# moss-lab/ScanFold

Hardware: AMD Instinct MI355X
Metric: windows/sec (W=120, step=1, 100 shuffles) (higher is better)
Workload: dtype int32 (int16 LDS storage) energies; f64 partition function

## Files before the change

### scanfold_amd/csrc/scanfold_hip.hip

```cpp
#include <math.h>
#include <stddef.h>
#include <stdio.h>
#include <stdlib.h>
#include <string.h>

#include <algorithm>
#include <map>
#include <string>
#include <vector>

#include "../../include/scanfold_hip_long.h"
#include "sf_launch.h"
#include "sf_energy.h"
#include "sf_mfe_full.hip.h"
#include "sf_mfe_fast.hip.h"
#include "sf_mfe_long.hip.h"
#include "sf_pf.hip.h"
#include "sf_pf_long.hip.h"
#include "sf_pf_fast.hip.h"
#include "sf_pf_lds.hip.h"
#include "sf_shuffle.hip.h"
#include "sf_tabulate.hip.h"
#include "sf_duplex.hip.h"

// ... 918 lines not shown
  return SF_OK;
}

int sf_last_status(void) {
  SF_ENTER();
  return read_status(nullptr, true);
}

int sf_set_max_bp_span(int span) {
  SF_ENTER();
  g.max_bp_span = span > 0 ? span : 0;
  if (g.have_params) {
    const int32_t md = g.max_bp_span > 0 ? g.max_bp_span - 1 : 0x7fffffff;
    HIPCHK(hipStreamSynchronize(g.stream));
    HIPCHK(hipMemcpy((char *)g.dP + offsetof(SfDevParams, max_pair_dist), &md, sizeof md, hipMemcpyHostToDevice));
    g.slot[g.cur].span = g.max_bp_span;
  }
  return SF_OK;
}

int sf_set_kernel_mode(int mode) {
  SF_ENTER();
  if (mode < 0 || mode > 1) return SF_ERR_BAD_ARG;
  g.force_full = (mode == 1);
  return SF_OK;
}


int sf_prof_reset(void) {
  SF_ENTER();
  HIPCHK(hipDeviceSynchronize());
  for (auto &e : g.ev) { hipEventDestroy(e.first); hipEventDestroy(e.second); }
  g.ev.clear();
  g.prof_ms = 0.0;
  g.prof_launches = 0;
  g.prof_folds = 0;
  g.prof_on = true;
  return SF_OK;
}

int sf_prof_get(double *ms, int64_t *launches, int64_t *folds) {
  SF_ENTER();
  HIPCHK(hipDeviceSynchronize());
  ProfPair::prof_drain();
  if (ms) *ms = g.prof_ms;
  if (launches) *launches = g.prof_launches;
  if (folds) *folds = g.prof_folds;
  return SF_OK;
}

int sf_prof_stop(void) {
  SF_ENTER();
  g.prof_on = false;
  return SF_OK;
}

}

namespace {
double g_long_ms[3] = {0, 0, 0};

struct LongBufs {
  std::vector<void *> ptrs;
  hipEvent_t ev[4] = {nullptr, nullptr, nullptr, nullptr};
  const char *who = "sf_fold_long";
  ~LongBufs() {
    hipStreamSynchronize(g.stream);
    for (void *p : ptrs) hipFree(p);
    for (hipEvent_t e : ev)
      if (e) hipEventDestroy(e);
  }
  int alloc(void **p, size_t bytes, const char *what) {
    *p = nullptr;
    const hipError_t e = hipMalloc(p, bytes ? bytes : 1);
    if (e != hipSuccess) {
      hipGetLastError();
      char b[512];
      snprintf(b, sizeof b, "%s: hipMalloc of %zu bytes (%s) failed: %s", who, bytes, what, hipGetErrorString(e));
      g.last_hip_error = b;
      *p = nullptr;
      return SF_ERR_HIP;
    }
    ptrs.push_back(*p);
    return SF_OK;
  }
};

int long_group(int d) {
  int G = 1;
  while (G < 64 && G * 64 < d) G *= 2;
  return G;
}
}

extern "C" {

int sf_fold_long(const uint8_t *seq, int L, const char *cons, int32_t *mfe_out, char *db_out) {
  int rc = check_ready();
  if (rc) return rc;
  if (!seq || L < 1 || L > SF_MAX_LONG) return SF_ERR_BAD_ARG;
  bool noncanonical = false;
  if (cons && (rc = scan_constraints(seq, cons, 1, L, &noncanonical))) return rc;
  const sf_params_blob *P = (const sf_params_blob *)g.slot[g.cur].src.data();
  std::vector<uint8_t> hS((size_t)L + 2, 0);
  for (int x = 0; x < L; x++) hS[x + 1] = sf_encode_nt(seq[x]);
  std::vector<int32_t> hhp((size_t)L + 1);
// ... 543 lines not shown
```

### scanfold_amd/csrc/sf_mfe_fast.hip.h

```cpp
#pragma once
#include <type_traits>
#include "sf_energy.h"
#include "sf_pk16.h"

#define SF_FAST_NR 34
#ifndef SF_FAST_TINY_D0
#define SF_FAST_TINY_D0 10
#endif
#define SF_FAST_CHUNK_D0 36
#ifndef SF_FAST_UNPACK
#define SF_FAST_UNPACK 1
#endif
#ifndef SF_UNP_PB
#define SF_UNP_PB 4
#endif
#define SF_HELP_MERGE_MAXW 118
#define SF_DML_HELPER_BIAS_256 26
#define SF_DML_HELPER_BIAS_W200 50
#define SF_DML_HELPER_BIAS(ng, wt) ((ng) == 256 ? ((wt) == 200 ? SF_DML_HELPER_BIAS_W200 : SF_DML_HELPER_BIAS_256) : 100000)
#define SF_HELP_NB_128 4
#define SF_HELP_NB_128G 8
#define SF_HELP_NB_256 6
#define SF_INF16 30000
#define SF_FAST_THRESH 10000
// ... 689 lines not shown
    if (!FOLD && slotd == 0) X.CI[SF_FAST_NR * RW + i0] = X.CI[rbd];
    const uint32_t bn = sf_pk(c + tau_in, c + X.t1n[SF_TIDX(tr, sq1, sp1)]);
    sf_fast_publish_bn(X.BN + 2 * rbd, i0, bn);
    if (X.bn_dup && slotd == 0) sf_fast_publish_bn(X.BN + 2 * (SF_FAST_NR * RW + i0), i0, bn);
    int stem, ext;
    if (i > 1 && j < W) { stem = X.tM[SF_TIDX(type, sp1, sq1)]; ext = X.tE[SF_TIDX(type, sp1, sq1)]; }
    else if (i > 1) stem = ext = X.tD5[type * 5 + sp1];
    else if (j < W) stem = ext = X.tD3[type * 5 + sq1];
    else stem = ext = 0;
    f = c + stem + tau_in + X.MLintern;
    cx = sfd_min(c + ext + tau_in, SF_INF16);
  } else {
    X.CI[rbd] = SF_INF16; sf_fast_publish_bn(X.BN + 2 * rbd, i0, sf_pk(SF_INF16, SF_INF16));
    if (!FOLD && slotd == 0) X.CI[SF_FAST_NR * RW + i0] = SF_INF16;
    if (X.bn_dup && slotd == 0) sf_fast_publish_bn(X.BN + 2 * (SF_FAST_NR * RW + i0), i0, sf_pk(SF_INF16, SF_INF16));
  }
  X.cg[SF_CGIDX(i, j)] = (int16_t)cx;
  if (final_fml && d > SFD_TURN + 1) f = sfd_min(f, fnb);
  if ((SEC & SF_SEC_DML) && (SEC & SF_SEC_FIN)) multiloop_split();
  f = sfd_min(f, dec);
  dprev = dec > SF_FAST_THRESH ? SF_INF16 : dec;
  fpart = f;
  if (final_fml && f < SF_FAST_OVF) ovf = 1;
  X.fML[FBASE(d) + i0] = (int16_t)(f > SF_FAST_THRESH ? SF_INF16 : f);
#undef ROW
#undef ROWB_CI
#undef ROWB_BN
#undef CIROW
#undef BNROWB
}

__device__ __forceinline__ int sf_wave_min(int v) {
#ifdef SF_EMUL
  return sfemul_wave_min(v);
#else
  v = sfd_min(v, __builtin_amdgcn_update_dpp(v, v, 0xB1, 0xF, 0xF, false));
  v = sfd_min(v, __builtin_amdgcn_update_dpp(v, v, 0x4E, 0xF, 0xF, false));
  v = sfd_min(v, __builtin_amdgcn_update_dpp(v, v, 0x141, 0xF, 0xF, false));
  v = sfd_min(v, __builtin_amdgcn_update_dpp(v, v, 0x140, 0xF, 0xF, false));
  v = sfd_min(v, __builtin_amdgcn_update_dpp(v, v, 0x142, 0xA, 0xF, false));
  v = sfd_min(v, __builtin_amdgcn_update_dpp(v, v, 0x143, 0xC, 0xF, false));
  return __builtin_amdgcn_readlane(v, 63);
#endif
}

__device__ __forceinline__ uint32_t sf_wave_next(uint32_t v) {
#ifdef SF_EMUL
  return __shfl_down(v, 1);
#else
  return (uint32_t)__builtin_amdgcn_update_dpp(0, (int)v, 0x130, 0xF, 0xF, true);
#endif
}

template <int WT, int LGC = 0>
__device__ __forceinline__ int sf_fast_dml2(const SfFastCtx &X, const int d, const int lane, const int i_own, const bool valid) {
  constexpr bool FOLD = false;
  const int W = WT ? WT : X.W;
  const int n = W - d, npairs = (n + 1) >> 1;
  const int lg = LGC ? LGC : (npairs <= 7 ? 3 : (npairs <= 15 ? 4 : 5));
  const int NC = 64 >> lg;
  const int q = lane & ((1 << lg) - 1), c = lane >> lg;
  const int elast = (d & 1) ? d - 6 : d - 5;
  const int N = elast - 3;
  const int S = (((N + NC - 1) >> (6 - lg)) + 1) & ~1;
  const int T8 = (S + 7) & ~7;
  const int ms = sfd_min(4 + c * S, elast - T8 + 1);
  const int ys = d - 1 - ms;
  const int par_a = W & 1, M0 = W - ys, par_b = (W - d + 1) & 1;
  const char *pa = (const char *)(X.fML + FBASE(ms) + 2 * q) - 36;
  const char *pb = (const char *)(X.fML + FBASE(ys) + 2 * q + ms + 1) - 64;
  int sa0 = 2 * (W - ms + par_a), sa1 = sa0 - 4 * par_a;
  int sb0 = 2 * (M0 - 1 - par_b), sb1 = 2 * (M0 - 1 + par_b);
  uint32_t acc0 = sf_pk(32767, 32767), acc1 = acc0;
  for (int t = 0; t < T8; t += 8) {
    uint32_t wa[8], wb[8];
#pragma unroll
    for (int k = 0; k < 8; k++) {
      constexpr int E[8] = {0, 0, 0, 2, 4, 8, 12, 18}, G2[8] = {0, 2, 4, 8, 12, 18, 24, 32};
      wa[k] = sf_ldw((const int16_t *)(pa + (36 - 2 * E[k])));
      wb[k] = sf_ldw((const int16_t *)(pb + (64 - 2 * G2[k] - ((k & 1) ? 0 : 2))));
      pa += (k & 1) ? (k < 7 ? sa1 : sa1 - 48) : sa0;
      pb -= (k & 1) ? (k < 7 ? sb1 : sb1 + 80) : sb0;
    }
    sa0 -= 16; sa1 -= 16; sb0 += 16; sb1 += 16;
#pragma unroll
    for (int k = 0; k < 8; k++) {
      uint32_t b = wb[k];
      if (!(k & 1)) b = (sf_wave_next(b) << 16) | (b >> 16);
      if (k & 1) acc1 = sf_pkmin(acc1, sf_pkadd(wa[k], b)); else acc0 = sf_pkmin(acc0, sf_pkadd(wa[k], b));
    }
  }
  if (d & 1) {
    const uint32_t a = sf_ldw(X.fML + FBASE(d - 5) + 2 * q);
    const uint32_t w = sf_ldw(X.fML + 2 * q + d - 5);
    acc0 = sf_pkmin(acc0, sf_pkadd(a, (sf_wave_next(w) << 16) | (w >> 16)));
  }
  uint32_t acc = sf_pkmin(acc0, acc1);
  acc = sf_pkmin_xor32(acc);
  if (lg <= 4) acc = sf_pkmin_xor16(acc);
  if (lg <= 3) acc = sf_pkmin_xor8(acc);
  const int i0 = valid ? i_own - 1 : 0;
  const uint32_t r = __shfl(acc, i0 >> 1);
  return (i0 & 1) ? sf_hi(r) : sf_lo(r);
}

__device__ __forceinline__ int sf_fast_c(const SfFastCtx &X, const int16_t *tExt, const int i, const int j) {
  const int W = X.W;
  const int v = X.cg[SF_CGIDX(i, j)];
  if (!X.cg_ext || v >= SF_INF16) return v;
  const uint8_t *S = X.S;
  const int type = X.tPair[S[i] * 8 + S[j]];
  int ext;
  if (i > 1 && j < W) ext = tExt[SF_TIDX(type, S[i - 1], S[j + 1])];
  else if (i > 1) ext = X.tD5[type * 5 + S[i - 1]];
  else if (j < W) ext = X.tD3[type * 5 + S[j + 1]];
  else ext = 0;
  return v - ext - (type > 2 ? X.TAU : 0);
}

__device__ inline int sf_fast_traceback(const SfFastCtx &X, const int32_t *f5s, const int16_t *tExt, const int lane,
                                        int16_t *stI, int16_t *stJ, int16_t *stM, char *dbL) {
  const int W = X.W;
  const bool FOLD = X.fold != 0;
  const uint8_t *S = X.S;
  const SfDevParams *D = X.D;
#define TC(i, j) sf_fast_c(X, tExt, (i), (j))
#define TF(i, j) (((j) - (i) < SFD_TURN + 1) ? SF_INF16 : (int)X.fML[FBASE((j) - (i)) + (i)-1])
#define TPAIR(i, j) (((j) - (i)) <= X.maxd ? (int)X.tPair[S[i] * 8 + S[j]] : 0)
  for (int x = lane; x < W; x += 64) dbL[x] = '.';
  int sp = 0, bad = 0;
  stI[0] = 1; stJ[0] = (int16_t)W; stM[0] = 0; sp = 1;
  while (sp > 0 && !bad) {
    --sp;
    int i = stI[sp], j = stJ[sp];
    const int ml = stM[sp];
    bool have_pair = false;
    if (ml == 0) {
      while (j > 0 && f5s[j] == f5s[j - 1]) j--;
      if (j < SFD_TURN + 2) continue;
      const int fij = f5s[j];
      int found = -1;
      for (int base = j - SFD_TURN - 1; base >= 1 && found < 0; base -= 64) {
        const int k = base - lane;
        bool ok = false;
        if (k >= 1) {
          const int type = TPAIR(k, j);
          if (type) {
            int ext;
            if (k > 1 && j < W) ext = tExt[SF_TIDX(type, S[k - 1], S[j + 1])];
            else if (k > 1) ext = X.tD5[type * 5 + S[k - 1]];
            else if (j < W) ext = X.tD3[type * 5 + S[j + 1]];
            else ext = 0;
            ok = (fij == f5s[k - 1] + TC(k, j) + ext + (type > 2 ? X.TAU : 0));
          }
        }
// ... 194 lines not shown
    if (bad && lane == 0) atomicOr(status, 1);
  }
}

#define SF_DEFER_ROWS_256 3
template <int NQ>
struct SfTrail {
  int F[NQ];
  int f3n;
  int row;
};
template <int NQ>
__device__ __forceinline__ void sf_trail_load(const int16_t *cgp, const int W, const int lane, const int i, int (&c)[NQ]) {
#pragma unroll
  for (int q = 0; q < NQ; q++) {
    const int j = lane + 1 + 64 * q;
    c[q] = (i >= 1 && j <= W && i + SFD_TURN + 1 <= j) ? (int)cgp[SF_CGIDX(i, j)] : SF_INF16;
  }
}
template <int NQ>
__device__ __forceinline__ void sf_trail_row(SfTrail<NQ> &T, const int lane, const int i, const int (&c)[NQ]) {
  if (i < 1) return;
  int m = c[0] + T.F[0];
#pragma unroll
  for (int q = 1; q < NQ; q++) m = sfd_min(m, c[q] + T.F[q]);
  T.f3n = sfd_min(T.f3n, sf_wave_min(m));
  if (i >= 2) {
    const int l = (i - 2) & 63, h = (i - 2) >> 6;
#pragma unroll
    for (int q = 0; q < NQ; q++) T.F[q] = (lane == l && h == q) ? T.f3n : T.F[q];
  }
}
template <int NQ, int NR>
__device__ __forceinline__ void sf_trail_rows(SfTrail<NQ> &T, const int lane, const int nrows, const int (&c)[NR][NQ]) {
#pragma unroll
  for (int k = 0; k < NR; k++)
    if (k < nrows) sf_trail_row<NQ>(T, lane, T.row - k, c[k]);
  T.row -= nrows;
}
template <int NQ>
__device__ __forceinline__ void sf_trail_result(const SfTrail<NQ> &T, const int lane, const int seq, const int over,
                                                int32_t *__restrict__ out, int *__restrict__ ovf_cnt,
                                                int *__restrict__ ovf_list) {
  if (lane == 0) {
    out[seq] = T.f3n;
    if (over || T.f3n < SF_FAST_OVF) {
      const int k = atomicAdd(ovf_cnt, 1);
      ovf_list[k] = seq;
    }
  }
}


enum SfStep {
  SF_STEP_SIZED,
  SF_STEP_GUARDED,
  SF_STEP_UNSPLIT,
  SF_STEP_SPLIT,
  SF_STEP_SPLIT16,
  SF_STEP_SPLIT8,
  SF_STEP_NARROW,
};
template <SfStep K>
using SfStepTag = std::integral_constant<SfStep, K>;

__device__ __forceinline__ int16_t sf_poison16(const int poison, const int x) {
  const int k = poison == 5 ? 1 + (int)(((uint32_t)x * 2654435761u) >> 30) : poison;
  return (int16_t)(k == 1 ? -32768 : (k == 2 ? -28000 : (k == 3 ? 0 : 32767)));
}

template <int NG, int WT, bool MG = false, bool HC = false, bool PZ = false>
__global__ __launch_bounds__(2 * NG, SF_FAST_WAVES_PER_SIMD) void sf_mfe_fast_kernel(const uint8_t *__restrict__ seqs, int n, int Wrt,
                                                             const SfDevParams *__restrict__ D,
                                                             const SfFastParams *__restrict__ F,
                                                             const SfFastRows *__restrict__ Rows,
                                                             int16_t *__restrict__ cg_all, int32_t *__restrict__ out,
                                                             int *__restrict__ ovf_cnt, int *__restrict__ ovf_list,
                                                             int trace_stride, char *__restrict__ db_out,
                                                             int *__restrict__ status, int *__restrict__ work_ctr,
                                                             const char *__restrict__ cons_rows,
                                                             const int32_t *__restrict__ sc_rows, int poison) {
  constexpr int NT = 2 * NG;
  constexpr bool FOLD = (NG == 256);
  const int W = WT ? WT : Wrt;
  SF_DYN_SMEM(smem);
  const SfFastLayout Lo = sf_fast_layout(W, HC);
  SfFastCtx X;
  char *const hcC = (char *)(smem + Lo.off_hc);
  uint8_t *const hcP = (uint8_t *)hcC + (W + 2), *const hcE = hcP + (W + 2);
  int16_t *const scS = (int16_t *)(smem + Lo.off_hc + (((3 * (W + 2)) + 1) & ~1));
  X.hc.c = (HC && cons_rows) ? hcC : nullptr; X.hc.partner = hcP; X.hc.encl = hcE;
  X.sc = (HC && sc_rows) ? scS : nullptr;
  X.fML = (int16_t *)smem;
  X.CI = (int16_t *)(smem + Lo.off_ci);
  X.C1N = nullptr; X.CB = nullptr;
  X.BN = (int16_t *)(smem + Lo.off_c1n);
#ifdef SF_EMUL
  sf_emul_bn_base = (const char *)X.BN; sf_emul_ci_base = (const char *)X.CI;
#endif
  X.DMLr = nullptr;
  int16_t *tab = (int16_t *)(smem + Lo.off_tab);
  X.t23 = tab; X.tI = tab + 175 - 25; X.t1n = tab + 325 - 25; X.tM = tab + 475 - 25; X.tH = tab + 625 - 25;
  X.tE = tab + 775 - 25; X.cg_ext = 1;
  X.tStack = tab + 925; X.tD5 = tab + 989; X.tD3 = tab + 1029;
  uint8_t *tPair = (uint8_t *)(tab + 1069);
  X.tPair = tPair;
  uint8_t *tRPair = (uint8_t *)(tab + SF_FAST_TAB_OLD);
  int16_t *t23in = tab + SF_FAST_TAB_OLD + 32;
  X.tRPair = tRPair; X.t23in = t23in;
  int32_t *flag = (int32_t *)(smem + Lo.off_flag);
  uint8_t *S = (uint8_t *)(smem + Lo.off_S);
  X.S = S;
  X.D = D; X.F = F; X.R = Rows; X.W = W; X.fold = FOLD; X.maxd = D->max_pair_dist;
  constexpr bool MERGE = MG && (NG == 128);
  constexpr bool UNPK = SF_FAST_UNPACK && (NG == 128);
  constexpr bool LGLOOPS = MG && (NG == 128);
  constexpr int TBLK = WT > 0 ? 1 : (NG == 128 ? (MG ? 2 : 1) : 0);
  X.bn_dup = (NG == 128);
  uint8_t *const cell_list = (MG && W >= SF_HELP_MERGE_MAXW) ? (uint8_t *)((int16_t *)(smem + Lo.off_tab) + 1069 + 32 + 1)
                                                            : (uint8_t *)(smem + Lo.off_list);
  X.TAU = D->P.TerminalAU; X.MLbase = D->P.MLbase; X.MLclosing = D->P.MLclosing; X.MLintern = D->P.MLintern[1];
  int32_t *f5s = (int32_t *)(smem + Lo.off_ci);
  int16_t *tExt = (int16_t *)(smem + Lo.off_ci + (((W + 1) * 4 + 3) & ~3));

  const int tid = threadIdx.x;
  X.cg = cg_all + (size_t)sf_fast_scratch_slot(blockIdx.x, gridDim.x) * SF_CG_ENTRIES(W);
  for (int x = tid; x < 175; x += NT) {
    tab[x] = F->mm23[x];
    if (x < 150) {
      tab[175 + x] = F->mmI[25 + x]; tab[325 + x] = F->mm1n[25 + x]; tab[475 + x] = F->mmM[25 + x];
      tab[625 + x] = F->mmH[25 + x]; tab[775 + x] = F->mmExt[25 + x];
    }
  }
  for (int x = tid; x < 175; x += NT) t23in[x] = F->mm23in[x];
  for (int x = tid; x < 64; x += NT) { tab[925 + x] = F->stackT[x]; tPair[x] = F->pair[x]; tRPair[x] = F->rpair[x]; }
  for (int x = tid; x < 40; x += NT) { tab[989 + x] = F->d5[x]; tab[1029 + x] = F->d3[x]; }

  {
    int16_t *uni = tab + 1069 + 32 + 1;
    X.uNIN = uni;
    for (int x = tid; x < 128; x += NT) uni[x] = F->uni[x];
  }
  const int grp = SF_WAVE_UNIFORM(tid / NG);
  const int tg = tid - grp * NG;
  constexpr int CENTRE = (NG == 256) ? 128 : 32;
  constexpr bool SHARE = SF_DML_HELPER_BIAS(NG, WT) < 10000;
  constexpr bool DML2 = (NG == 128);
  const int OFFs = ((W + 1) >> 1) - CENTRE;
  const int OFF = (NG > 64) ? (OFFs + NG) & (NG - 1) : 0;
  const int v = (tg + OFF) & (NG - 1);
  constexpr int MAIN_LO = (NG == 256) ? 64 : 0, MAIN_HI = (NG == 256) ? 191 : 63;
  const bool can_split = (NG == 128 && W >= 64) || NG == 256;
  const int split_d0 = can_split ? ((sfd_max(sfd_max(SFD_MAXLOOP + 6, 2 * (MAIN_LO - 1 + OFFs)), 2 * (W - OFFs - MAIN_HI)) + 1) & ~1) : 1 << 30;
  constexpr bool NARROW = (NG == 256);
  const int narrow_d0 = (NARROW && can_split && W >= 168)
                            ? sfd_max(split_d0, (sfd_max(2 * (96 - 1 + OFFs), 2 * (W - OFFs - 159)) + 1) & ~1) : 1 << 30;

  constexpr int NQ = NG / 64;
  const bool sweeper = SF_WAVE_UNIFORM(tid >> 6) == (NG == 128 ? 3 : 7);
  const int n_split_steps = split_d0 < W ? (W - split_d0 + 1) / 2 : 0;
  constexpr int DROWS = (NG == 128 || WT != 200) ? 4 : SF_DEFER_ROWS_256;
  const int defer_need = n_split_steps > 0 ? (W - SFD_TURN - 1 + n_split_steps - 1) / n_split_steps : 0;
  const int defer_rows = sfd_min(defer_need, DROWS);
  const bool defer_on = n_split_steps >= 8 && defer_need <= 4;
  SfTrail<NQ> T;
#pragma unroll
  for (int q = 0; q < NQ; q++) T.F[q] = 0;
  T.f3n = 0; T.row = 0;

  int *const next_slot = (int *)(smem + Lo.off_next);
  int seq = blockIdx.x;
  while (seq < n) {
    const uint8_t *src = seqs + (size_t)seq * W;
    constexpr bool PINF = true;
    int tidf = tid;
    if (PINF) SF_PIN(tidf);
    __syncthreads();
    if (PZ) {
      for (int x = tid; x < Lo.off_tab / 2; x += NT) ((int16_t *)smem)[x] = sf_poison16(poison, x);
      if (HC) for (int x = tid; x < (Lo.total - Lo.off_hc) / 2; x += NT) ((int16_t *)(smem + Lo.off_hc))[x] = sf_poison16(poison, x);
      __syncthreads();
    }
    for (int x = tidf; x < W; x += NT) S[x + 1] = sf_encode_nt(src[x]);
    if (MG && W >= SF_HELP_MERGE_MAXW) for (int x = tidf; x < 128; x += NT) ((int16_t *)(smem + Lo.off_tab) + 1069 + 32 + 1)[x] = F->uni[x];
    for (int x = tidf; x < (Lo.off_tab - Lo.off_ci) / 4; x += NT) ((uint32_t *)X.CI)[x] = sf_pk(SF_INF16, SF_INF16);
    int fetched = 0;
    if (tid == 0) {
      S[0] = 0; S[W + 1] = 0; flag[0] = 0;
      fetched = (int)gridDim.x + atomicAdd(work_ctr, 1);
    }
    __syncthreads();
    if (HC) {
      if (cons_rows)
        for (int x = tid; x < W; x += NT) hcC[x + 1] = cons_rows[(size_t)seq * W + x];
      if (sc_rows)
        for (int x = tid; x < W; x += NT) scS[x + 1] = (int16_t)sfd_max(sfd_min(sc_rows[(size_t)seq * W + x], 30000), -30000);
      __syncthreads();
      if (cons_rows && tid == 0) flag[0] = sf_hc_parse8(W, hcC, hcP, hcE) ? 2 : 0;
      __syncthreads();
      if (cons_rows && flag[0] == 2) {
        if (tid == 0) { atomicOr(status, 2); out[seq] = 0; *next_slot = fetched; }
        __syncthreads();
        seq = *next_slot;
        continue;
      }
    }
    int next_seq = n;
    const bool trail_this = defer_on && !(db_out && (seq % trace_stride) == 0);
    if (sweeper) {
#pragma unroll
      for (int q = 0; q < NQ; q++) T.F[q] = 0;
      T.f3n = 0; T.row = trail_this ? W - SFD_TURN - 1 : 0;
    }
    int ovf = 0;
    uint32_t H[14];
    int dprev = SF_INF16;
    int fnb = SF_FAST_BIG;
#pragma unroll
    for (int k = 0; k < 14; k++) H[k] = (uint32_t)SF_INF16 | ((uint32_t)SF_INF16 << 16);

    int slot2 = (SFD_TURN + 1 + grp - 2) % SF_FAST_NR, slotd = (SFD_TURN + 1 + grp) % SF_FAST_NR;
    auto build_list = [&](const int dd0) {
      const int lane = tid & 63;
      const int d1 = dd0 + 1;
      const int iH = ((v - 64) & (NG - 1)) - (dd0 >> 1);
      const bool vA = (dd0 < W) && (iH >= 1) && (iH + dd0 <= W), vB = (d1 < W) && (iH >= 1) && (iH + d1 <= W);
      const int tA = (vA && dd0 <= X.maxd) ? X.tPair[S[iH] * 8 + S[iH + dd0]] : 0;
      const int tB = (vB && d1 <= X.maxd) ? X.tPair[S[iH] * 8 + S[iH + d1]] : 0;
      const unsigned long long mA = __ballot(tA != 0), mB = __ballot(tB != 0);
      const int cA = __popcll(mA);
      uint8_t *list = cell_list + (((dd0 >> 1) & 1) << 7);
      const unsigned long long below = (1ull << lane) - 1ull;
      if (tA) list[__popcll(mA & below)] = (uint8_t)iH;
      if (tB) list[cA + __popcll(mB & below)] = (uint8_t)(iH | 128);
      if (lane == 0) list[127] = (uint8_t)(cA + __popcll(mB));
    };
    SfHU HU;
    auto step = [&](const int d0, auto kind_tag) {
      constexpr SfStep KIND = decltype(kind_tag)::value;
      constexpr int LGC = KIND == SF_STEP_SPLIT16 ? 4 : (KIND == SF_STEP_SPLIT8 ? 3 : (KIND == SF_STEP_SPLIT && LGLOOPS ? 5 : 0));
      constexpr bool DO_G = KIND == SF_STEP_SIZED, DO_CH = KIND == SF_STEP_GUARDED;
      const int d = d0 + grp;
      if (d0 == SFD_TURN + 1 + 2 && tid == 0) *next_slot = fetched;
      if (d0 == SFD_TURN + 1 + 4) next_seq = SF_WAVE_UNIFORM(*next_slot);
      constexpr bool split = KIND >= SF_STEP_SPLIT;
      constexpr bool narrow = KIND == SF_STEP_NARROW;
      if (NARROW && d0 == narrow_d0) {
        uint32_t *const xa = (uint32_t *)X.BN;
        const int RWc = W - 4;
        if (tg >= 96 && tg < 160) {
#pragma unroll
          for (int k = 0; k < 14; k++) xa[(grp * 16 + k) * RWc + 100 + (tg - 96)] = H[k];
          xa[(grp * 16 + 14) * RWc + 100 + (tg - 96)] = (uint32_t)dprev;
          xa[(grp * 16 + 15) * RWc + 100 + (tg - 96)] = (uint32_t)fnb;
        }
        __syncthreads();
        if (tg >= 64 && tg < 128) {
#pragma unroll
          for (int k = 0; k < 14; k++) H[k] = xa[(grp * 16 + k) * RWc + 100 + (tg - 64)];
          dprev = (int)xa[(grp * 16 + 14) * RWc + 100 + (tg - 64)];
          fnb = (int)xa[(grp * 16 + 15) * RWc + 100 + (tg - 64)];
        }
        __syncthreads();
      }
      const bool helper = split && (NG == 256 ? (narrow ? tg < 64 : (tg < 64 || tg >= 192)) : tg >= 64);
      const int vh = NG == 256 ? (narrow ? v + 96 : (tg < 64 ? v + 64 : v - 64)) : v - 64;
      const int vm = narrow ? ((v + 32) & (NG - 1)) : v;
      constexpr bool DML4 = NARROW && (WT == 200);
      const bool dmlw = DML4 && narrow && tg >= 128;
      const int vd = tg >= 192 ? v - 96 : v - 32;
      const int i = (NARROW && !DML4 && narrow && tg >= 128) ? -1
                    : ((dmlw ? (vd & (NG - 1)) : (helper ? (vh & (NG - 1)) : vm)) - (d >> 1));
      const int dml_terms = d - 2 * SFD_TURN - 2;
      const int dml_cut = d - SFD_TURN - 1 - sfd_max(sfd_min(dml_terms / 2 - SF_DML_HELPER_BIAS(NG, WT), dml_terms), 0);
      const bool valid = (d < W) && (i >= 1) && (i + d <= W);
      int fpart = SF_FAST_BIG;
      int dec = SF_FAST_BIG, eh = SF_FAST_BIG, e0 = SF_FAST_BIG;
      SfPub pub;
      pub.a = pub.b = 0; pub.tau = 0; pub.type = 0;
      int dc[DROWS][NQ];
      const bool sweep_now = defer_on && sweeper && split && T.row > 0;
      const int sweep_rows = sweep_now ? sfd_max(sfd_min(defer_rows, T.row - (W - d0)), 0) : 0;
      if (sweep_now) {
#pragma unroll
        for (int k = 0; k < DROWS; k++)
          if (k < sweep_rows) sf_trail_load<NQ>(X.cg, W, tid & 63, T.row - k, dc[k]);
      }
      if (__ballot(valid)) {
        if (DO_G && d0 < 8) sf_fast_cell<true, WT, SF_SEC_ALL, false, FOLD, 1>(X, d, i, valid, slot2, slotd, H, HU, ovf, grp == 0, fnb, fpart, dec, eh, e0, dprev, pub);
        else if (DO_G && d0 < SF_FAST_TINY_D0) sf_fast_cell<true, WT, SF_SEC_ALL, false, FOLD, 5>(X, d, i, valid, slot2, slotd, H, HU, ovf, grp == 0, fnb, fpart, dec, eh, e0, dprev, pub);
        else if (DO_CH && d0 < SF_FAST_CHUNK_D0) sf_fast_cell<false, WT, SF_SEC_ALL, true, FOLD, SFD_MAXLOOP, TBLK>(X, d, i, valid, slot2, slotd, H, HU, ovf, grp == 0, fnb, fpart, dec, eh, e0, dprev, pub);
        else if (!split) sf_fast_cell<false, WT, SF_SEC_ALL, false, FOLD, SFD_MAXLOOP, TBLK, false, UNPK && KIND == SF_STEP_UNSPLIT>(X, d, i, valid, slot2, slotd, H, HU, ovf, grp == 0, fnb, fpart, dec, eh, e0, dprev, pub);
        else if (DML4 && narrow) {
          const int nmain = dml_terms / 5, cA = SFD_TURN + 1 + nmain, cB = cA + (dml_terms - nmain + 1) / 2;
          uint32_t *const xa = (uint32_t *)X.BN;
          if (dmlw) {
            const bool wB = tg >= 192;
            sf_fast_cell<false, WT, SF_SEC_DML, false, FOLD, SFD_MAXLOOP, TBLK>(X, d, i, valid, slot2, slotd, H, HU, ovf, false, fnb, fpart, dec, eh, e0, dprev, pub, wB ? cB : cA, wB ? (1 << 20) : cB - 1);
            if (valid) xa[(grp * 16 + (wB ? 1 : 0)) * (W - 4) + 100 + (tg & 63)] = (uint32_t)sfd_min(dec, 32000);
          } else if (!helper) {
            sf_fast_cell<false, WT, SF_SEC_P1 | SF_SEC_C0 | SF_SEC_DML | SF_SEC_PRE, false, FOLD, SFD_MAXLOOP, TBLK>(X, d, i, valid, slot2, slotd, H, HU, ovf, grp == 0, fnb, fpart, dec, eh, e0, dprev, pub, SFD_TURN + 1, cA - 1);
          } else {
            sf_fast_cell<false, WT, SF_SEC_HELP, false, FOLD, SFD_MAXLOOP, TBLK>(X, d, i, valid, slot2, slotd, H, HU, ovf, grp == 0, fnb, fpart, dec, eh, e0, dprev, pub);
            if (valid) X.BN[2 * (slotd * (W - 4) + i - 1)] = (int16_t)sfd_min(eh, 32000);
          }
        }
        else if (!helper) {
          if (SHARE) sf_fast_cell<false, WT, SF_SEC_P1 | SF_SEC_C0 | SF_SEC_DML | SF_SEC_PRE, false, FOLD, SFD_MAXLOOP, TBLK>(X, d, i, valid, slot2, slotd, H, HU, ovf, grp == 0, fnb, fpart, dec, eh, e0, dprev, pub, SFD_TURN + 1, dml_cut - 1);
          else {
            static_assert(SHARE || DML2, "a main wave either shares the multiloop split with its helpers (NG = 256) or runs it two cells per lane (NG = 128)");
            dec = sf_fast_dml2<WT, LGC>(X, d, tid & 63, i, valid);
            sf_fast_cell<false, WT, SF_SEC_P1 | SF_SEC_C0 | SF_SEC_PRE, false, FOLD, SFD_MAXLOOP, TBLK, false, UNPK && split>(X, d, i, valid, slot2, slotd, H, HU, ovf, grp == 0, fnb, fpart, dec, eh, e0, dprev, pub);
          }
        } else if (MERGE) {
          const int lane = tid & 63;
          const uint8_t *list = cell_list + (((d0 >> 1) & 1) << 7);
          const int cT = SF_WAVE_UNIFORM((int)list[127]);
          const int e = (grp << 6) + lane;
          if (SF_WAVE_UNIFORM(cT > (grp << 6))) {
            const bool vC = e < cT;
            const int ent = vC ? list[e] : 1;
            const int g = ent >> 7, iC = ent & 127;
            const int s2 = slot2 - grp < 0 ? slot2 - grp + SF_FAST_NR : slot2 - grp;
            const int sd0 = slotd - grp < 0 ? slotd - grp + SF_FAST_NR : slotd - grp;
            const int sd1 = sd0 + 1 >= SF_FAST_NR ? 0 : sd0 + 1;
            SfFastCtx Xh = X;
            Xh.BN = X.BN + 2 * g * (W - 4);
            sf_fast_cell<false, WT, SF_SEC_HELP, false, FOLD, SFD_MAXLOOP, TBLK, true>(Xh, d0 + g, iC, vC, s2, sd0, H, HU, ovf, false, fnb, fpart, dec, eh, e0, dprev, pub);
            if (vC) X.BN[2 * ((g ? sd1 : sd0) * (W - 4) + iC - 1)] = (int16_t)sfd_min(eh, 32000);
          }
        } else {
          if (SHARE) {
            sf_fast_cell<false, WT, SF_SEC_HELP | SF_SEC_DML, false, FOLD, SFD_MAXLOOP, TBLK>(X, d, i, valid, slot2, slotd, H, HU, ovf, grp == 0, fnb, fpart, dec, eh, e0, dprev, pub, dml_cut);
            if (valid) {
              X.BN[2 * (slotd * (W - 4) + i - 1)] = (int16_t)sfd_min(eh, 32000);
              X.CI[slotd * (W - 4) + i - 1] = (int16_t)sfd_min(dec, 32000);
            }
          } else {
            sf_fast_cell<false, WT, SF_SEC_HELP, false, FOLD, SFD_MAXLOOP, TBLK>(X, d, i, valid, slot2, slotd, H, HU, ovf, grp == 0, fnb, fpart, dec, eh, e0, dprev, pub);
            if (valid) X.BN[2 * (slotd * (W - 4) + i - 1)] = (int16_t)sfd_min(eh, 32000);
          }
        }
      }
      if (sweep_now && sweep_rows > 0) sf_trail_rows<NQ, DROWS>(T, tid & 63, sweep_rows, dc);
      if (MERGE && grp == 1 && tg >= 64 && d0 + 2 >= split_d0 && d0 + 2 < W) build_list(d0 + 2);
      if (split) {
        __syncthreads();
        if (!helper && !dmlw && __ballot(valid)) {
          if (valid) {
            eh = X.BN[2 * (slotd * (W - 4) + i - 1)];
            if (DML4 && narrow) {
              const uint32_t *const xa = (const uint32_t *)X.BN;
              dec = sfd_min(dec, sfd_min((int)xa[(grp * 16) * (W - 4) + 100 + (tg & 63)], (int)xa[(grp * 16 + 1) * (W - 4) + 100 + (tg & 63)]));
            } else if (SHARE) dec = sfd_min(dec, (int)X.CI[slotd * (W - 4) + i - 1]);
          }
          sf_fast_cell<false, WT, SF_SEC_FIN | SF_SEC_POST, false, FOLD, SFD_MAXLOOP, TBLK>(X, d, i, valid, slot2, slotd, H, HU, ovf, grp == 0, fnb, fpart, dec, eh, e0, dprev, pub);
        }
      }
      __syncthreads();
      if (grp == 0 && valid && !helper && !dmlw) {
        const int d1 = d0 + 1;
        const int16_t *pd = X.fML + FBASE(d1), *pe = X.fML + FBASE(d0);
        const bool ex0 = i + d1 <= W, ex1 = i >= 2;
        const int ia = i - 1, ib = ex1 ? i - 2 : 0;
        const int p0 = pd[ia], p1 = pd[ib], q0 = pe[i], q1 = pe[ia], q2 = pe[ib];
        const int v0 = sfd_min(p0, sfd_min(q0, q1) + X.MLbase), v1 = sfd_min(p1, sfd_min(q1, q2) + X.MLbase);
        if ((ex0 && v0 < SF_FAST_OVF) || (ex1 && v1 < SF_FAST_OVF)) ovf = 1;
        const int g0 = (ex0 && v0 <= SF_FAST_THRESH) ? v0 : SF_INF16, g1 = (ex1 && v1 <= SF_FAST_THRESH) ? v1 : SF_INF16;
        if (ex0) X.fML[FBASE(d1) + ia] = (int16_t)g0;
        fnb = sfd_min(g0, g1) + X.MLbase;
      }
      slot2 += 2; if (slot2 >= SF_FAST_NR) slot2 -= SF_FAST_NR;
      slotd += 2; if (slotd >= SF_FAST_NR) slotd -= SF_FAST_NR;
    };
    {
      int d0 = SFD_TURN + 1;
      for (; d0 < SF_FAST_TINY_D0 && d0 < W; d0 += 2) step(d0, SfStepTag<SF_STEP_SIZED>{});
      for (; d0 < SF_FAST_CHUNK_D0 && d0 < W; d0 += 2) step(d0, SfStepTag<SF_STEP_GUARDED>{});
      if constexpr (UNPK) {
#pragma unroll
        for (int x = 0; x < 27; x++) HU.v[x] = (short)((x & 1) ? (H[x >> 1] >> 16) : (H[x >> 1] & 0xffffu));
      }
      for (; d0 < split_d0 && d0 < W; d0 += 2) step(d0, SfStepTag<SF_STEP_UNSPLIT>{});
      if constexpr (LGLOOPS) {
        for (; d0 < W - 30 && d0 < W; d0 += 2) step(d0, SfStepTag<SF_STEP_SPLIT>{});
        for (; d0 < W - 14 && d0 < W; d0 += 2) step(d0, SfStepTag<SF_STEP_SPLIT16>{});
        for (; d0 < W; d0 += 2) step(d0, SfStepTag<SF_STEP_SPLIT8>{});
      }
      for (; d0 < (NARROW ? narrow_d0 : W) && d0 < W; d0 += 2) step(d0, SfStepTag<SF_STEP_SPLIT>{});
      if constexpr (NARROW)
        for (; d0 < W; d0 += 2) step(d0, SfStepTag<SF_STEP_NARROW>{});
    }

    if (ovf) flag[0] = 1;
    if (trail_this) {
      __syncthreads();
      if (sweeper) {
        while (T.row >= 1) {
          int tc[4][NQ];
#pragma unroll
          for (int k = 0; k < 4; k++) sf_trail_load<NQ>(X.cg, W, tid & 63, T.row - k, tc[k]);
          sf_trail_rows<NQ, 4>(T, tid & 63, sfd_min(4, T.row), tc);
        }
        sf_trail_result<NQ>(T, tid & 63, seq, flag[0], out, ovf_cnt, ovf_list);
      }
    } else {
    int tidn = tid;
    if (PINF && WT != 120) SF_PIN(tidn);
    for (int x = tidn; x < 200; x += NT) tExt[x] = F->mmExt[x];
    __syncthreads();
    int16_t *etab = nullptr;
    if (tid < 64)
      sf_fast_exterior<NG / 64>(X, W, tidn, seq, f5s, tExt, etab, flag, (int16_t *)(smem + Lo.off_cb),
                      (char *)(smem + Lo.off_cb + ((3 * (W + 8) * 2 + 3) & ~3)), out, ovf_cnt, ovf_list, trace_stride,
                      db_out, status);
    }
    seq = next_seq;
  }
#undef FBASE
#undef FLEN
}

#define SF_FAST_INSTANCES(X)                                                                          \
  X(128, 0, false, false, false) X(128, 0, true, false, false) X(128, 120, true, false, false)        \
  X(256, 200, false, false, false) X(256, 0, false, false, false)                                     \
  X(128, 0, false, true, false) X(128, 0, true, true, false) X(256, 0, false, true, false)            \
  X(128, 0, false, false, true) X(128, 0, true, false, true) X(128, 120, true, false, true)           \
  X(256, 200, false, false, true) X(256, 0, false, false, true)
struct SfFastInstance {
  int ng, wt;
  bool mg, hc, pz;
};
static inline SfFastInstance sf_fast_select(int W, bool hc, bool pz) {
  SfFastInstance s;
  s.ng = sf_fast_threads(W) / 2;
  s.wt = (!hc && (W == 120 || W == 200)) ? W : 0;
  s.mg = s.wt == 120 || W < SF_HELP_MERGE_MAXW;
  s.hc = hc;
  s.pz = pz;
  return s;
// ... 41 lines not shown
```

### scanfold_amd/csrc/sf_pk16.h

```cpp
#pragma once
#include <stdint.h>
#include <string.h>
#include "sf_launch.h"

#ifdef SF_EMUL
static inline uint32_t sf_pk(int lo, int hi) { return ((uint32_t)lo & 0xffffu) | ((uint32_t)hi << 16); }
static inline int sf_lo(uint32_t p) { return (int)(int16_t)(p & 0xffffu); }
static inline int sf_hi(uint32_t p) { return (int)(int16_t)(p >> 16); }
static inline int sf_sat16(int v) { return v > 32767 ? 32767 : (v < -32768 ? -32768 : v); }
static inline uint32_t sf_pkmin(uint32_t a, uint32_t b) {
  return sf_pk(sf_lo(a) < sf_lo(b) ? sf_lo(a) : sf_lo(b), sf_hi(a) < sf_hi(b) ? sf_hi(a) : sf_hi(b));
}
static inline uint32_t sf_pkadd(uint32_t a, uint32_t b) {
  return sf_pk(sf_sat16(sf_lo(a) + sf_lo(b)), sf_sat16(sf_hi(a) + sf_hi(b)));
}
static inline uint32_t sf_ldw(const int16_t *p) {
  if ((uintptr_t)p & 3) { fprintf(stderr, "sf_mfe_pk: misaligned dword access\n"); abort(); }
  uint32_t v; memcpy(&v, p, 4); return v;
}
static inline void sf_stw(int16_t *p, uint32_t v) {
  if ((uintptr_t)p & 3) { fprintf(stderr, "sf_mfe_pk: misaligned dword access\n"); abort(); }
  memcpy(p, &v, 4);
}
static inline void sf_store_fence() {}
#else
typedef short sf_s2 __attribute__((ext_vector_type(2)));
__device__ __forceinline__ uint32_t sf_pk(int lo, int hi) { return ((uint32_t)lo & 0xffffu) | ((uint32_t)hi << 16); }
__device__ __forceinline__ int sf_lo(uint32_t p) { return (int)(int16_t)(p & 0xffffu); }
__device__ __forceinline__ int sf_hi(uint32_t p) { return (int)p >> 16; }
__device__ __forceinline__ uint32_t sf_pkmin(uint32_t a, uint32_t b) {
  return __builtin_bit_cast(uint32_t, __builtin_elementwise_min(__builtin_bit_cast(sf_s2, a), __builtin_bit_cast(sf_s2, b)));
}
__device__ __forceinline__ uint32_t sf_pkadd(uint32_t a, uint32_t b) {
  return __builtin_bit_cast(uint32_t, __builtin_elementwise_add_sat(__builtin_bit_cast(sf_s2, a), __builtin_bit_cast(sf_s2, b)));
}
__device__ __forceinline__ uint32_t sf_ldw(const int16_t *p) { return *(const uint32_t *)p; }
__device__ __forceinline__ void sf_stw(int16_t *p, uint32_t v) { *(uint32_t *)p = v; }
__device__ __forceinline__ void sf_store_fence() { asm volatile("" ::: "memory"); }
#endif
#ifdef SF_EMUL
static inline uint32_t sf_pkmin_xor32(uint32_t v) { return sf_pkmin(v, (uint32_t)__shfl_xor((int)v, 32)); }
static inline uint32_t sf_pkmin_xor16(uint32_t v) { return sf_pkmin(v, (uint32_t)__shfl_xor((int)v, 16)); }
static inline uint32_t sf_pkmin_xor8(uint32_t v) { return sf_pkmin(v, (uint32_t)__shfl_xor((int)v, 8)); }
#else
__device__ __forceinline__ uint32_t sf_pkmin_xor32(uint32_t v) {
  const auto r = __builtin_amdgcn_permlane32_swap(v, v, false, false);
  return sf_pkmin(r[0], r[1]);
}
__device__ __forceinline__ uint32_t sf_pkmin_xor16(uint32_t v) {
  const auto r = __builtin_amdgcn_permlane16_swap(v, v, false, false);
  return sf_pkmin(r[0], r[1]);
}
__device__ __forceinline__ uint32_t sf_pkmin_xor8(uint32_t v) {
  return sf_pkmin(v, (uint32_t)__builtin_amdgcn_update_dpp((int)v, (int)v, 0x128, 0xF, 0xF, false));
}
#endif
#ifdef SF_EMUL
static inline short sf_opaque16(short x) { return x; }
#else
__device__ __forceinline__ short sf_opaque16(short x) { asm("" : "+v"(x)); return x; }
#endif
__device__ __forceinline__ uint32_t sf_ld2(const int16_t *p, const int odd) {
  if (odd) {
    const uint32_t d0 = sf_ldw(p - 1), d1 = sf_ldw(p + 1);
    return (d0 >> 16) | (d1 << 16);
  }
  return sf_ldw(p);
}
__device__ __forceinline__ uint32_t sf_ld2r(const int16_t *p, const int odd) {
  const uint32_t d0 = sf_ldw(p - odd), d1 = sf_ldw(p - odd + 2);
  return (uint32_t)((((uint64_t)d1 << 32) | d0) >> (odd << 4));
}
__device__ __forceinline__ void sf_st2(int16_t *p, const int odd, uint32_t v) {
  if (odd) {
    p[0] = (int16_t)(v & 0xffffu);
    sf_store_fence();
    p[1] = (int16_t)(v >> 16);
  } else {
    sf_stw(p, v);
  }
}
```

Before: 44540.

## Refine multiloop split lane geometry with non-power-of-two lane groups and finer tails

Reworks the two-cell-per-lane multiloop (dml2) split so the per-diagonal lane group size follows the remaining row count more closely. It adds 21-, 12-, 4- and 2-lane groupings, with a cross-chunk reduction done through ds_bpermute fetches for the non-power-of-two cases, and lets the term count round to a multiple of 4 via a trailing half batch. The goal is to cut wasted multiloop terms and idle lanes near the end of each window's diagonals. The cost is more step specialisations, which means more code, possible register pressure, and extra permute traffic in the 21- and 12-lane reductions. A host-side geometry query function is also added for testing.

```diff
diff --git a/scanfold_amd/csrc/scanfold_hip.hip b/scanfold_amd/csrc/scanfold_hip.hip
--- a/scanfold_amd/csrc/scanfold_hip.hip
+++ b/scanfold_amd/csrc/scanfold_hip.hip
@@ -994,6 +994,16 @@
 int sf_prof_stop(void) {
   SF_ENTER();
   g.prof_on = false;
+  return SF_OK;
+}
+
+int sf_dml2_geometry(int W, int hc, int d, int lane, int32_t *out) {
+  if (!out || W < 1 || W > 128 || lane < 0 || lane > 63) return SF_ERR_BAD_ARG;
+  const int d0 = sf_fast_split_d0<128>(W);
+  if (d < d0 || d >= W) return SF_ERR_BAD_ARG;
+  const SfDml2Geom G = sf_dml2_geom<0>(W, d, lane, sf_fast_select(W, hc != 0, false).mg);
+  out[0] = G.lanes; out[1] = G.chunks; out[2] = G.share; out[3] = G.terms; out[4] = G.last; out[5] = G.c; out[6] = G.q;
+  out[7] = G.first;
   return SF_OK;
 }
 
diff --git a/scanfold_amd/csrc/sf_mfe_fast.hip.h b/scanfold_amd/csrc/sf_mfe_fast.hip.h
--- a/scanfold_amd/csrc/sf_mfe_fast.hip.h
+++ b/scanfold_amd/csrc/sf_mfe_fast.hip.h
@@ -765,19 +765,66 @@
 #endif
 }
 
-template <int WT, int LGC = 0>
+
+struct SfDml2Geom {
+  int lanes;
+  int chunks;
+  int share;
+  int terms;
+  int last;
+  int c, q;
+  int first;
+};
+__host__ __device__ __forceinline__ int sf_dml2_lanes(const int W, const int d, const bool np2) {
+  const int n0 = W - (d & ~1);
+  return n0 <= 2 ? 2 : (n0 <= 6 ? 4 : (n0 <= 14 ? 8 : (np2 && n0 <= 22 ? 12 : (n0 <= 30 ? 16 : (np2 && n0 <= 40 ? 21 : 32)))));
+}
+template <int LANES = 0>
+__host__ __device__ __forceinline__ SfDml2Geom sf_dml2_geom(const int W, const int d, const int lane, const bool np2) {
+  SfDml2Geom G;
+  G.lanes = LANES ? LANES : sf_dml2_lanes(W, d, np2);
+  G.last = (d & 1) ? d - 6 : d - 5;
+  const int N = G.last - 3;
+  int per;
+  if (LANES == 21 || LANES == 12) {
+    G.chunks = 64 / (LANES ? LANES : 1);
+    G.c = (lane * (2048 / (LANES ? LANES : 1) + 1)) >> 11;
+    G.q = lane - G.c * LANES;
+    per = (N + G.chunks - 1) / G.chunks;
+  } else if (!LANES && np2 && (G.lanes == 21 || G.lanes == 12)) {
+    G.chunks = 64 / G.lanes;
+    G.c = lane / G.lanes;
+    G.q = lane - G.c * G.lanes;
+    per = (N + G.chunks - 1) / G.chunks;
+  } else {
+    const int lg = G.lanes == 32 ? 5 : (G.lanes == 16 ? 4 : (G.lanes == 8 ? 3 : (G.lanes == 4 ? 2 : 1)));
+    G.chunks = 64 >> lg;
+    G.c = lane >> lg;
+    G.q = lane & (G.lanes - 1);
+    per = (N + G.chunks - 1) >> (6 - lg);
+  }
+  G.share = (per + 1) & ~1;
+  G.terms = (G.share + 3) & ~3;
+  const int lo = 4 + G.c * G.share, hi = G.last - G.terms + 1;
+  G.first = lo < hi ? lo : hi;
+  return G;
+}
+
+__device__ __forceinline__ uint32_t sf_lane_fetch(const uint32_t v, const int src) {
+#ifdef SF_EMUL
+  return (uint32_t)__shfl((int)v, src);
+#else
+  return (uint32_t)__builtin_amdgcn_ds_bpermute(src << 2, (int)v);
+#endif
+}
+
+template <int WT, int LANES = 0, bool NP2 = false>
 __device__ __forceinline__ int sf_fast_dml2(const SfFastCtx &X, const int d, const int lane, const int i_own, const bool valid) {
   constexpr bool FOLD = false;
   const int W = WT ? WT : X.W;
-  const int n = W - d, npairs = (n + 1) >> 1;
-  const int lg = LGC ? LGC : (npairs <= 7 ? 3 : (npairs <= 15 ? 4 : 5));
-  const int NC = 64 >> lg;
-  const int q = lane & ((1 << lg) - 1), c = lane >> lg;
-  const int elast = (d & 1) ? d - 6 : d - 5;
-  const int N = elast - 3;
-  const int S = (((N + NC - 1) >> (6 - lg)) + 1) & ~1;
-  const int T8 = (S + 7) & ~7;
-  const int ms = sfd_min(4 + c * S, elast - T8 + 1);
+  const SfDml2Geom G = sf_dml2_geom<LANES>(W, d, lane, NP2);
+  const int q = G.q, T = G.terms;
+  const int ms = G.first;
   const int ys = d - 1 - ms;
   const int par_a = W & 1, M0 = W - ys, par_b = (W - d + 1) & 1;
   const char *pa = (const char *)(X.fML + FBASE(ms) + 2 * q) - 36;
@@ -785,35 +832,53 @@
   int sa0 = 2 * (W - ms + par_a), sa1 = sa0 - 4 * par_a;
   int sb0 = 2 * (M0 - 1 - par_b), sb1 = 2 * (M0 - 1 + par_b);
   uint32_t acc0 = sf_pk(32767, 32767), acc1 = acc0;
-  for (int t = 0; t < T8; t += 8) {
-    uint32_t wa[8], wb[8];
-#pragma unroll
-    for (int k = 0; k < 8; k++) {
+  auto batch = [&](auto nb_tag) {
+    constexpr int NB = decltype(nb_tag)::value;
+    uint32_t wa[NB], wb[NB];
+#pragma unroll
+    for (int k = 0; k < NB; k++) {
       constexpr int E[8] = {0, 0, 0, 2, 4, 8, 12, 18}, G2[8] = {0, 2, 4, 8, 12, 18, 24, 32};
       wa[k] = sf_ldw((const int16_t *)(pa + (36 - 2 * E[k])));
       wb[k] = sf_ldw((const int16_t *)(pb + (64 - 2 * G2[k] - ((k & 1) ? 0 : 2))));
-      pa += (k & 1) ? (k < 7 ? sa1 : sa1 - 48) : sa0;
-      pb -= (k & 1) ? (k < 7 ? sb1 : sb1 + 80) : sb0;
-    }
-    sa0 -= 16; sa1 -= 16; sb0 += 16; sb1 += 16;
-#pragma unroll
-    for (int k = 0; k < 8; k++) {
+      if (k + 1 < NB || NB == 8) {
+        pa += (k & 1) ? (k < 7 ? sa1 : sa1 - 48) : sa0;
+        pb -= (k & 1) ? (k < 7 ? sb1 : sb1 + 80) : sb0;
+      }
+    }
+    if (NB == 8) { sa0 -= 16; sa1 -= 16; sb0 += 16; sb1 += 16; }
+#pragma unroll
+    for (int k = 0; k < NB; k++) {
       uint32_t b = wb[k];
       if (!(k & 1)) b = (sf_wave_next(b) << 16) | (b >> 16);
       if (k & 1) acc1 = sf_pkmin(acc1, sf_pkadd(wa[k], b)); else acc0 = sf_pkmin(acc0, sf_pkadd(wa[k], b));
     }
-  }
+  };
+  for (int t = 8; t <= T; t += 8) batch(std::integral_constant<int, 8>{});
+  if (T & 4) batch(std::integral_constant<int, 4>{});
   if (d & 1) {
     const uint32_t a = sf_ldw(X.fML + FBASE(d - 5) + 2 * q);
     const uint32_t w = sf_ldw(X.fML + 2 * q + d - 5);
     acc0 = sf_pkmin(acc0, sf_pkadd(a, (sf_wave_next(w) << 16) | (w >> 16)));
   }
   uint32_t acc = sf_pkmin(acc0, acc1);
-  acc = sf_pkmin_xor32(acc);
-  if (lg <= 4) acc = sf_pkmin_xor16(acc);
-  if (lg <= 3) acc = sf_pkmin_xor8(acc);
   const int i0 = valid ? i_own - 1 : 0;
-  const uint32_t r = __shfl(acc, i0 >> 1);
+  uint32_t r;
+  if (LANES == 21 || LANES == 12) {
+    constexpr int NC = 64 / (LANES ? LANES : 1);
+    uint32_t f[NC];
+#pragma unroll
+    for (int c = 0; c < NC; c++) f[c] = sf_lane_fetch(acc, (i0 >> 1) + c * LANES);
+    r = f[0];
+#pragma unroll
+    for (int c = 1; c < NC; c++) r = sf_pkmin(r, f[c]);
+  } else {
+    acc = sf_pkmin_xor32(acc);
+    if (G.lanes <= 16) acc = sf_pkmin_xor16(acc);
+    if (G.lanes <= 8) acc = sf_pkmin_xor8(acc);
+    if (G.lanes <= 4) acc = sf_pkmin_xor4(acc);
+    if (G.lanes <= 2) acc = sf_pkmin_xor2(acc);
+    r = sf_lane_fetch(acc, i0 >> 1);
+  }
   return (i0 & 1) ? sf_hi(r) : sf_lo(r);
 }
 
@@ -1114,6 +1179,16 @@
 }
 
 
+template <int NG>
+__host__ __device__ __forceinline__ int sf_fast_split_d0(const int W) {
+  constexpr int CENTRE = (NG == 256) ? 128 : 32, MAIN_LO = (NG == 256) ? 64 : 0, MAIN_HI = (NG == 256) ? 191 : 63;
+  const int OFFs = ((W + 1) >> 1) - CENTRE;
+  const bool can_split = (NG == 128 && W >= 64) || NG == 256;
+  const int a = SFD_MAXLOOP + 6, b = 2 * (MAIN_LO - 1 + OFFs), c = 2 * (W - OFFs - MAIN_HI);
+  const int m = a > b ? (a > c ? a : c) : (b > c ? b : c);
+  return can_split ? ((m + 1) & ~1) : 1 << 30;
+}
+
 enum SfStep {
   SF_STEP_SIZED,
   SF_STEP_GUARDED,
@@ -1121,6 +1196,10 @@
   SF_STEP_SPLIT,
   SF_STEP_SPLIT16,
   SF_STEP_SPLIT8,
+  SF_STEP_SPLIT21,
+  SF_STEP_SPLIT12,
+  SF_STEP_SPLIT4,
+  SF_STEP_SPLIT2,
   SF_STEP_NARROW,
 };
 template <SfStep K>
@@ -1213,7 +1292,7 @@
   const int v = (tg + OFF) & (NG - 1);
   constexpr int MAIN_LO = (NG == 256) ? 64 : 0, MAIN_HI = (NG == 256) ? 191 : 63;
   const bool can_split = (NG == 128 && W >= 64) || NG == 256;
-  const int split_d0 = can_split ? ((sfd_max(sfd_max(SFD_MAXLOOP + 6, 2 * (MAIN_LO - 1 + OFFs)), 2 * (W - OFFs - MAIN_HI)) + 1) & ~1) : 1 << 30;
+  const int split_d0 = sf_fast_split_d0<NG>(W);
   constexpr bool NARROW = (NG == 256);
   const int narrow_d0 = (NARROW && can_split && W >= 168)
                             ? sfd_max(split_d0, (sfd_max(2 * (96 - 1 + OFFs), 2 * (W - OFFs - 159)) + 1) & ~1) : 1 << 30;
@@ -1300,7 +1379,8 @@
     SfHU HU;
     auto step = [&](const int d0, auto kind_tag) {
       constexpr SfStep KIND = decltype(kind_tag)::value;
-      constexpr int LGC = KIND == SF_STEP_SPLIT16 ? 4 : (KIND == SF_STEP_SPLIT8 ? 3 : (KIND == SF_STEP_SPLIT && LGLOOPS ? 5 : 0));
+      constexpr int LANES = KIND == SF_STEP_SPLIT21 ? 21 : (KIND == SF_STEP_SPLIT16 ? 16 : (KIND == SF_STEP_SPLIT12 ? 12 : (KIND == SF_STEP_SPLIT8 ? 8
+                            : (KIND == SF_STEP_SPLIT4 ? 4 : (KIND == SF_STEP_SPLIT2 ? 2 : (KIND == SF_STEP_SPLIT && LGLOOPS ? 32 : 0))))));
       constexpr bool DO_G = KIND == SF_STEP_SIZED, DO_CH = KIND == SF_STEP_GUARDED;
       const int d = d0 + grp;
       if (d0 == SFD_TURN + 1 + 2 && tid == 0) *next_slot = fetched;
@@ -1371,7 +1451,7 @@
           if (SHARE) sf_fast_cell<false, WT, SF_SEC_P1 | SF_SEC_C0 | SF_SEC_DML | SF_SEC_PRE, false, FOLD, SFD_MAXLOOP, TBLK>(X, d, i, valid, slot2, slotd, H, HU, ovf, grp == 0, fnb, fpart, dec, eh, e0, dprev, pub, SFD_TURN + 1, dml_cut - 1);
           else {
             static_assert(SHARE || DML2, "a main wave either shares the multiloop split with its helpers (NG = 256) or runs it two cells per lane (NG = 128)");
-            dec = sf_fast_dml2<WT, LGC>(X, d, tid & 63, i, valid);
+            dec = sf_fast_dml2<WT, LANES, LGLOOPS>(X, d, tid & 63, i, valid);
             sf_fast_cell<false, WT, SF_SEC_P1 | SF_SEC_C0 | SF_SEC_PRE, false, FOLD, SFD_MAXLOOP, TBLK, false, UNPK && split>(X, d, i, valid, slot2, slotd, H, HU, ovf, grp == 0, fnb, fpart, dec, eh, e0, dprev, pub);
           }
         } else if (MERGE) {
@@ -1445,9 +1525,13 @@
       }
       for (; d0 < split_d0 && d0 < W; d0 += 2) step(d0, SfStepTag<SF_STEP_UNSPLIT>{});
       if constexpr (LGLOOPS) {
-        for (; d0 < W - 30 && d0 < W; d0 += 2) step(d0, SfStepTag<SF_STEP_SPLIT>{});
-        for (; d0 < W - 14 && d0 < W; d0 += 2) step(d0, SfStepTag<SF_STEP_SPLIT16>{});
-        for (; d0 < W; d0 += 2) step(d0, SfStepTag<SF_STEP_SPLIT8>{});
+        for (; d0 < W - 40 && d0 < W; d0 += 2) step(d0, SfStepTag<SF_STEP_SPLIT>{});
+        for (; d0 < W - 30 && d0 < W; d0 += 2) step(d0, SfStepTag<SF_STEP_SPLIT21>{});
+        for (; d0 < W - 22 && d0 < W; d0 += 2) step(d0, SfStepTag<SF_STEP_SPLIT16>{});
+        for (; d0 < W - 14 && d0 < W; d0 += 2) step(d0, SfStepTag<SF_STEP_SPLIT12>{});
+        for (; d0 < W - 6 && d0 < W; d0 += 2) step(d0, SfStepTag<SF_STEP_SPLIT8>{});
+        for (; d0 < W - 2 && d0 < W; d0 += 2) step(d0, SfStepTag<SF_STEP_SPLIT4>{});
+        for (; d0 < W; d0 += 2) step(d0, SfStepTag<SF_STEP_SPLIT2>{});
       }
       for (; d0 < (NARROW ? narrow_d0 : W) && d0 < W; d0 += 2) step(d0, SfStepTag<SF_STEP_SPLIT>{});
       if constexpr (NARROW)
diff --git a/scanfold_amd/csrc/sf_pk16.h b/scanfold_amd/csrc/sf_pk16.h
--- a/scanfold_amd/csrc/sf_pk16.h
+++ b/scanfold_amd/csrc/sf_pk16.h
@@ -42,6 +42,8 @@
 static inline uint32_t sf_pkmin_xor32(uint32_t v) { return sf_pkmin(v, (uint32_t)__shfl_xor((int)v, 32)); }
 static inline uint32_t sf_pkmin_xor16(uint32_t v) { return sf_pkmin(v, (uint32_t)__shfl_xor((int)v, 16)); }
 static inline uint32_t sf_pkmin_xor8(uint32_t v) { return sf_pkmin(v, (uint32_t)__shfl_xor((int)v, 8)); }
+static inline uint32_t sf_pkmin_xor4(uint32_t v) { return sf_pkmin(v, (uint32_t)__shfl_xor((int)v, 4)); }
+static inline uint32_t sf_pkmin_xor2(uint32_t v) { return sf_pkmin(v, (uint32_t)__shfl_xor((int)v, 2)); }
 #else
 __device__ __forceinline__ uint32_t sf_pkmin_xor32(uint32_t v) {
   const auto r = __builtin_amdgcn_permlane32_swap(v, v, false, false);
@@ -53,6 +55,12 @@
 }
 __device__ __forceinline__ uint32_t sf_pkmin_xor8(uint32_t v) {
   return sf_pkmin(v, (uint32_t)__builtin_amdgcn_update_dpp((int)v, (int)v, 0x128, 0xF, 0xF, false));
+}
+__device__ __forceinline__ uint32_t sf_pkmin_xor4(uint32_t v) {
+  return sf_pkmin(v, (uint32_t)__builtin_amdgcn_update_dpp((int)v, (int)v, 0x124, 0xF, 0xF, false));
+}
+__device__ __forceinline__ uint32_t sf_pkmin_xor2(uint32_t v) {
+  return sf_pkmin(v, (uint32_t)__builtin_amdgcn_update_dpp((int)v, (int)v, 0x4E, 0xF, 0xF, false));
 }
 #endif
 #ifdef SF_EMUL
```

After: 44530. Within noise of the previous version (-0.0%).
